# serenedb/serenedb

Measured on AMD Instinct MI355X. Metric: docs scored/sec BM25 top-1000 (+ rows/sec filter-agg), higher is better.
Workload: dtype f32; 1 GPU; bm25_top1000_4term_or_100M; execution=pipelined-batch, doc_count=100000000, k=1000, seed=43, postings_per_query=18005713, total_matches=17052989, parallelism=doc-range shards x1, RCCL allgather merge

## Files before the change

### serenedb_amd/csrc/hip/sdb_gpu.hip

```cpp

#include <hip/hip_runtime.h>

#include <algorithm>
#include <cfloat>
#include <cmath>
#include <cstdint>
#include <cstdlib>
#include <cstring>
#include <vector>
#include <chrono>
#include <cstdio>

#include "../../../include/sdb_gpu.h"
#include "sdb_internal.h"

#define SDB_TERM_SLOTS 64u
#ifndef SDB_WIN_DOCS
#define SDB_WIN_DOCS 24576u
#endif
#ifndef SDB_NTHREADS
#define SDB_NTHREADS 1024u
#endif
#define SDB_NWAVES (SDB_NTHREADS / 64u)
#define SDB_MAX_TERMS 32u
// ... 934 lines not shown
    }
    __syncthreads();
    SDB_T(4)
#endif
  }
  if (tid == 0 && wg_matches) atomicAdd(a.total_matches, wg_matches);
#ifdef SDB_TIMING
  if (tid == 0)
    for (int i = 0; i < 6; ++i)
      atomicAdd(&a.bucket_out[i], t_acc[i]);
#endif
}


struct SweepItem {
  uint32_t t;
  float num;
  const uint8_t* pl;
  SdbBlockDesc d;
};

template <uint32_t WD, uint32_t NTH, bool WIDE>
__launch_bounds__(NTH, NTH == 1024 ? 4 : 2) __global__
void topk_sweep_kernel(WindowArgs a, const TermDev* __restrict__ terms) {
  constexpr uint32_t NW = NTH / 64u;
  constexpr uint32_t NWORDS = WD / 64u;
  static_assert(WD - 1u < SDB_SLOT_ABSENT, "slot offsets are u16");
  extern __shared__ __attribute__((aligned(16))) char smem[];
  float* swin = (float*)smem;
  unsigned long long* mwin = (unsigned long long*)(swin + WD);
  uint32_t* scratch = (uint32_t*)(mwin + NWORDS);
  uint32_t* hist = scratch + NW * 384;
  uint32_t* shared_misc = hist + SDB_HIST_BINS;
  uint32_t* cursors = shared_misc + 2 + NW;
  float* wub = (float*)(cursors + SDB_MAX_TERMS);
  uint32_t* icnt = (uint32_t*)(wub + SDB_MAX_TERMS);
  uint32_t* iadv = icnt + SDB_MAX_TERMS;
  TermDev* tstage = (TermDev*)(iadv + SDB_MAX_TERMS);
  unsigned long long* lbuck =
    (unsigned long long*)(tstage + a.nterms);
  SdbBlockDesc* dcache =
    (SdbBlockDesc*)(lbuck + (a.fcol ? 2 * SDB_MAX_BUCKETS : 0u));
  const uint32_t stage_off =
    ((uint32_t)((char*)(dcache + a.nterms * a.dcache_n) - smem) + 15u) & ~15u;
  char* stage = smem + stage_off;
  const uint32_t C = a.round_items;

  const uint32_t tid = threadIdx.x;
  const int lane = tid & 63;
  const uint32_t wave = tid >> 6;
  for (uint32_t i = tid; i < a.nterms * (sizeof(TermDev) / 4); i += NTH)
    ((uint32_t*)tstage)[i] = ((const uint32_t*)terms)[i];
  const float inv_smax = (float)SDB_HIST_BINS / a.smax;
  uint32_t* gh = a.ghist + (blockIdx.x & 7u) * SDB_HIST_BINS;
  unsigned long long wg_matches = 0;
#ifdef SDB_TIMING
  unsigned long long t_acc[6] = {0, 0, 0, 0, 0, 0};
  long long t_mark = clock64();
#define SDB_TS(idx)                                        \
  if (tid == 0) {                                          \
    const long long now_ = clock64();                      \
    t_acc[idx] += (unsigned long long)(now_ - t_mark);     \
    t_mark = now_;                                         \
  }
#else
#define SDB_TS(idx)
#endif

  const uint32_t nwin = (a.doc_count + WD - 1) / WD;
  const uint32_t per = (nwin + gridDim.x - 1) / gridDim.x;
  const uint32_t w_lo = blockIdx.x * per;
  const uint32_t w_hi = min(nwin, w_lo + per);
  if (w_lo >= w_hi) return;

  __syncthreads();
  if (tid < a.nterms) {
    const TermDev te = tstage[tid];
    const uint32_t first_lo = 1u + w_lo * WD;
    cursors[tid] = (uint32_t)(
      lower_bound_last_doc(a.desc, te.desc_begin, te.desc_end, first_lo) -
      te.desc_begin);
  }
  __syncthreads();
  const float nc = tstage[0].nc, nl = tstage[0].nl;

  for (uint32_t w = w_lo; w < w_hi; ++w) {
    const uint32_t lo = 1u + w * WD;
    if (lo > a.doc_count) break;
    const uint32_t hi = min(lo + WD - 1u, a.doc_count);
    const uint32_t wlen = hi - lo + 1u;
    const bool derive = ((w & 3u) == 0) || (w < w_lo + 2);
    uint32_t my_excl_snap = 0;

    for (uint32_t t = wave; t < a.nterms; t += NW) {
      const TermDev te = tstage[t];
      uint64_t b = te.desc_begin + cursors[t] + (uint32_t)lane;
      uint32_t cnt = 0, adv = 0;
      for (;;) {
        uint32_t prev = 0xFFFFFFFFu, last = 0xFFFFFFFFu;
        if (b < te.desc_end) {
          prev = a.desc[b].prev_doc;
          last = a.desc[b].last_doc;
        }
        const uint32_t c = (uint32_t)__popcll(__ballot(prev < hi));
        adv += (uint32_t)__popcll(__ballot(last <= hi));
        cnt += c;
        if (c < 64u) break;
        b += 64u;
      }
      if (lane == 0) {
        icnt[t] = cnt;
        iadv[t] = adv;
      }
    }

    for (uint32_t i = tid; i < WD; i += NTH) swin[i] = 0.0f;
    for (uint32_t i = tid; i < NWORDS; i += NTH) mwin[i] = 0ull;
    if (derive)
      for (uint32_t i = tid; i < SDB_HIST_BINS; i += NTH) hist[i] = 0;
    if (a.fcol)
      for (uint32_t i = tid; i < 2 * a.nbuckets; i += NTH) lbuck[i] = 0;
    {
      const uint32_t words_per_term = a.dcache_n * 7u;
      for (uint32_t i = tid; i < a.nterms * words_per_term; i += NTH) {
        const uint32_t t = i / words_per_term;
        const uint32_t wrd = i % words_per_term;
        const TermDev te = tstage[t];
        const uint64_t b0 = te.desc_begin + cursors[t];
        const uint32_t avail =
          (uint32_t)(te.desc_end > b0 ? te.desc_end - b0 : 0);
        if (wrd < avail * 7u)
          ((uint32_t*)&dcache[t * a.dcache_n])[wrd] =
            ((const uint32_t*)&a.desc[b0])[wrd];
      }
    }
    if (tid == 0)
      shared_misc[0] = __hip_atomic_load(a.gthresh, __ATOMIC_RELAXED,
                                         __HIP_MEMORY_SCOPE_AGENT);
    if (a.wand) __syncthreads();
    if (a.wand) {
      for (uint32_t t = wave; t < a.nterms; t += NW) {
        const TermDev te = tstage[t];
        const uint32_t cur0w = cursors[t];
        float u = 0.0f;
        uint32_t beyond_f = 0;
        if ((uint32_t)lane < a.dcache_n &&
            te.desc_begin + cur0w + (uint32_t)lane < te.desc_end) {
          const SdbBlockDesc d = dcache[t * a.dcache_n + lane];
          if (d.prev_doc < hi)
            u = score_one(a.scorer, te.num, te.nc, te.nl, d.max_freq,
                          d.min_norm);
          else
            beyond_f = 1;
        }
#pragma unroll
        for (int o = 32; o; o >>= 1) u = fmaxf(u, __shfl_down(u, o, 64));
        const unsigned long long beyond = __ballot(beyond_f != 0);
        if (lane == 0) {
          float ub = u;
          if (!beyond) {
            for (uint64_t bb = te.desc_begin + cur0w + a.dcache_n;
                 bb < te.desc_end; ++bb) {
              const SdbBlockDesc d = a.desc[bb];
              if (d.prev_doc >= hi) break;
              const float uu = score_one(a.scorer, te.num, te.nc, te.nl,
                                         d.max_freq, d.min_norm);
              ub = uu > ub ? uu : ub;
            }
          }
          wub[t] = ub * a.fbmax * 1.0000019f;
        }
      }
    }
    __syncthreads();
    SDB_TS(0)
    float wand_total_ub = 0.0f;
    if (a.wand)
      for (uint32_t t = 0; t < a.nterms; ++t) wand_total_ub += wub[t];
    float gtw = 0.0f;
    if (a.wand && shared_misc[0]) {
      float t0 = (float)shared_misc[0] / inv_smax;
      uint32_t t0b;
      __builtin_memcpy(&t0b, &t0, 4);
      t0b = t0b > 2 ? t0b - 2 : 0;
      __builtin_memcpy(&gtw, &t0b, 4);
    }

    const uint32_t icnt_l = (uint32_t)lane < a.nterms ? icnt[lane] : 0u;
    const uint32_t ipre_incl = wave_incl_scan(icnt_l, lane);
    const uint32_t ipre_excl = ipre_incl - icnt_l;
    const uint32_t nitems =
      (uint32_t)__builtin_amdgcn_readlane((int)ipre_incl, 63);
    auto load_item = [&](uint32_t i, SweepItem& it) {
      const uint32_t t =
        (uint32_t)__builtin_ctzll(__ballot(ipre_incl > i));
      const uint32_t rel =
        i - (uint32_t)__builtin_amdgcn_readlane((int)ipre_excl, (int)t);
      const TermDev te = tstage[t];
      typedef __attribute__((address_space(3))) const uint32_t LdsWord;
      typedef __attribute__((address_space(1))) const uint32_t GlobalWord;
      uint32_t wv[10];
      if (rel < a.dcache_n) {
        LdsWord* p = (LdsWord*)&dcache[t * a.dcache_n + rel];
#pragma unroll
        for (int k = 0; k < 7; ++k) wv[k] = p[k];
      } else {
        GlobalWord* p =
          (GlobalWord*)&a.desc[te.desc_begin + cursors[t] + rel];
#pragma unroll
        for (int k = 0; k < 7; ++k) wv[k] = p[k];
      }
      __builtin_memcpy(wv + 7, &te.payload_begin, 8);
      __builtin_memcpy(wv + 9, &te.num, 4);
#pragma unroll
      for (int k = 0; k < 10; ++k)
        wv[k] = (uint32_t)__builtin_amdgcn_readfirstlane((int)wv[k]);
      uint64_t pbeg;
      __builtin_memcpy(&it.d, wv, 28);
      __builtin_memcpy(&pbeg, wv + 7, 8);
      __builtin_memcpy(&it.num, wv + 9, 4);
      it.t = t;
      it.pl = a.payload + pbeg;
// ... 90 lines not shown
        const uint32_t npair = (i1 - i0) * 64u;
        for (uint32_t p = tid; p < npair; p += NTH) {
          const char* sl = base + (p >> 6) * SDB_SLOT_BYTES;
          const uint32_t l = p & 63u;
          const float2 v = ((const float2*)sl)[l];
          const uint32_t o = ((const uint32_t*)(sl + 512))[l];
          const uint32_t o0 = o & 0xFFFFu, o1 = o >> 16;
          if (o0 != SDB_SLOT_ABSENT) swin_add(swin, o0, v.x);
          if (o1 != SDB_SLOT_ABSENT) swin_add(swin, o1, v.y);
        }
        __syncthreads();
      }
      SDB_TS(2)
    }
    if (tid < a.nterms) cursors[tid] += iadv[tid];

    uint32_t tbin_w = shared_misc[0];
    const uint32_t nw_act = (wlen + 63u) / 64u;
    uint32_t my_matches = 0;
    uint32_t my_cnt = 0;
    for (uint32_t i = tid; i < nw_act; i += NTH) {
      unsigned long long word = mwin[i];
      if (word && a.live) {
        const uint64_t d0 = (uint64_t)lo + 64u * i;
        const unsigned long long lw = (a.live[d0 >> 6] >> (d0 & 63u)) |
                                      (a.live[(d0 >> 6) + 1]
                                       << (64u - (d0 & 63u)));
        word &= lw;
        mwin[i] = word;
      }
      if (word && a.fcol) {
        unsigned long long w0 = word;
        while (w0) {
          const uint32_t bit = (uint32_t)__ffsll((long long)w0) - 1u;
          w0 &= w0 - 1;
          const uint32_t doc = lo + 64u * i + bit;
          const long long vv = a.fcol[doc];
          bool pass = vv >= a.flo && vv <= a.fhi;
          for (uint32_t x = 0; pass && x < a.nfx; ++x) {
            const long long xv = a.fxc[x][doc];
            if (a.fxop[x] == 1) pass = xv < a.fxlo[x];
            else if (a.fxop[x] == 2) pass = xv >= a.fxlo[x];
            else pass = (xv >= a.fxlo[x]) & (xv <= a.fxhi[x]);
          }
          if (!pass) {
            word &= ~(1ull << bit);
            continue;
          }
          const unsigned long long span_m1 =
            (unsigned long long)a.fhi - (unsigned long long)a.flo;
          const unsigned long long dv =
            (unsigned long long)vv - (unsigned long long)a.flo;
          const uint32_t bkt = WIDE
            ? sdb_bucket_wide(dv, a.nbuckets, span_m1)
            : sdb_bucket_narrow(dv, a.nbuckets, span_m1);
          atomicAdd(&lbuck[2 * bkt], 1ull);
          atomicAdd(&lbuck[2 * bkt + 1], (unsigned long long)vv);
        }
        mwin[i] = word;
      }
      if (!word) continue;
      my_matches += (uint32_t)__popcll(word);
      const uint32_t base = i * 64u;
      do {
        const uint32_t off = base + (uint32_t)__ffsll((long long)word) - 1u;
        word &= word - 1;
        const uint32_t sb = score_bin(swin[off], inv_smax);
        my_cnt += sb >= tbin_w ? 1u : 0u;
        if (derive) atomicAdd(&hist[sb], 1u);
      } while (word);
    }
    {
      const uint32_t incl0 = wave_incl_scan(my_cnt, lane);
      if (lane == 63) scratch[NTH + wave] = incl0;
      my_excl_snap = incl0 - my_cnt;
    }
    uint32_t wm = my_matches;
#pragma unroll
    for (int off = 32; off; off >>= 1) wm += __shfl_down(wm, off, 64);
    if (lane == 0) shared_misc[2 + wave] = wm;
    __syncthreads();
    SDB_TS(3)

    if (a.fcol)
      for (uint32_t i = tid; i < 2 * a.nbuckets; i += NTH)
        if (lbuck[i]) atomicAdd(&a.bucket_out[i], lbuck[i]);

    const uint32_t known_bin = __hip_atomic_load(
      a.gthresh, __ATOMIC_RELAXED, __HIP_MEMORY_SCOPE_AGENT);
    if (derive)
      for (uint32_t b = tid; b < SDB_HIST_BINS; b += NTH)
        if (b >= known_bin && hist[b]) atomicAdd(&gh[b], hist[b]);
    if (derive && wave == 0) {
      uint32_t part = 0;
      if (SDB_HIST_BINS - 1 - 4 * (uint32_t)lane + 3 >= known_bin) {
#pragma unroll
        for (int j = 0; j < 4; ++j) {
          const uint32_t b = SDB_HIST_BINS - 4 * lane - 4 + j;
#pragma unroll
          for (int sh = 0; sh < 8; ++sh)
            part += __hip_atomic_load(&a.ghist[sh * SDB_HIST_BINS + b],
                                      __ATOMIC_RELAXED,
                                      __HIP_MEMORY_SCOPE_AGENT);
        }
      }
      const uint32_t suff_incl = wave_incl_scan(part, lane);
      const uint32_t suff_prev = __shfl_up(suff_incl, 1, 64);
      const bool winner =
        suff_incl >= a.k && (lane == 0 || suff_prev < a.k);
      if (winner) {
        uint32_t cum = suff_incl - part;
        uint32_t binfloor = 0;
        for (int b = (int)(SDB_HIST_BINS - 1 - 4 * lane);; --b) {
          uint32_t add = 0;
#pragma unroll
          for (int sh = 0; sh < 8; ++sh)
            add += __hip_atomic_load(&a.ghist[sh * SDB_HIST_BINS + b],
                                     __ATOMIC_RELAXED,
                                     __HIP_MEMORY_SCOPE_AGENT);
          cum += add;
          if (cum >= a.k) {
            binfloor = (uint32_t)b;
            break;
          }
        }
        if (binfloor > known_bin) atomicMax(a.gthresh, binfloor);
      }
    }
    if (wave == 0 && lane == 0) {
      uint32_t total_m = 0;
      for (uint32_t v = 0; v < NW; ++v) total_m += shared_misc[2 + v];
      wg_matches += total_m;
    }
    SDB_TS(4)

    if (w == w_lo) {
      if (tid == 0)
        shared_misc[0] = __hip_atomic_load(a.gthresh, __ATOMIC_RELAXED,
                                           __HIP_MEMORY_SCOPE_AGENT);
      __syncthreads();
      tbin_w = shared_misc[0];
      uint32_t cnt2 = 0;
      for (uint32_t i = tid; i < nw_act; i += NTH) {
        unsigned long long word = mwin[i];
        if (!word) continue;
        const uint32_t base = i * 64u;
        do {
          const uint32_t off =
            base + (uint32_t)__ffsll((long long)word) - 1u;
          word &= word - 1;
          cnt2 += score_bin(swin[off], inv_smax) >= tbin_w ? 1u : 0u;
        } while (word);
      }
      const uint32_t incl2 = wave_incl_scan(cnt2, lane);
      if (lane == 63) scratch[NTH + wave] = incl2;
      my_excl_snap = incl2 - cnt2;
      __syncthreads();
    }

    uint32_t wave_base = 0;
    for (uint32_t v = 0; v < wave; ++v) wave_base += scratch[NTH + v];
    const uint32_t my_excl = wave_base + my_excl_snap;
    uint32_t block_total = 0;
    for (uint32_t v = 0; v < NW; ++v) block_total += scratch[NTH + v];
    if (tid == 0)
      shared_misc[1] =
        block_total ? atomicAdd(a.cand_count, block_total) : 0u;
    __syncthreads();
    const uint32_t cbase = shared_misc[1];
    if (cbase + block_total > a.cand_cap) {
      if (tid == 0) atomicExch(a.overflow, 1u);
      return;
    }
    uint32_t pos = cbase + my_excl;
    if (block_total)
      for (uint32_t i = tid; i < nw_act; i += NTH) {
        unsigned long long word = mwin[i];
        if (!word) continue;
        const uint32_t base = i * 64u;
        do {
          const uint32_t off =
            base + (uint32_t)__ffsll((long long)word) - 1u;
          word &= word - 1;
          const float s = swin[off];
          if (score_bin(s, inv_smax) >= tbin_w) {
            a.cands[pos].score = s;
            a.cands[pos].doc = lo + off;
            a.cands[pos].segment_idx = a.seg_idx;
            ++pos;
          }
        } while (word);
      }
    __syncthreads();
    SDB_TS(5)
  }
  if (tid == 0 && wg_matches) atomicAdd(a.total_matches, wg_matches);
#ifdef SDB_TIMING
  if (tid == 0)
    for (int i = 0; i < 6; ++i) atomicAdd(&a.bucket_out[i], t_acc[i]);
#endif
#undef SDB_TS
}



#ifndef SDB_PW_SUBW
#define SDB_PW_SUBW 1024u
#endif
#define SDB_PW_TERMS 4u
#define SDB_PW_NTH 256u

#ifndef SDB_PW_RING
#define SDB_PW_RING 256u
#endif
#ifndef SDB_PW_MINW
#define SDB_PW_MINW 2
#endif
#define SDB_PW_DSTAGE 8u
#define SDB_PW_WAVE_LDS_BYTES                                            \
  (SDB_PW_SUBW * 4  + (SDB_PW_SUBW / 64) * 8  +          \
   SDB_PW_TERMS * SDB_PW_RING * 8  + 384 * 4  +      \
   SDB_HIST_BINS * 4  +                                          \
   SDB_PW_TERMS * SDB_PW_DSTAGE * 28  + 32 )

struct PwState {
  uint64_t cur;
  uint64_t dend;
  uint64_t dsbase;
  uint64_t pbase;
  uint32_t ring_head;
  uint32_t ring_cnt;
  uint32_t cov;
  float num, nc, nl;
};

__device__ __forceinline__ uint32_t pw_fill_block(
  const WindowArgs& a, PwState& st, const SdbBlockDesc& d, int lane,
  uint32_t range_lo, uint32_t range_hi, unsigned long long* ring,
  uint32_t* scratch) {
  const uint8_t* pl = a.payload + st.pbase;
  uint32_t doc0 = 0, doc1 = 0;
  float s0 = 0.f, s1 = 0.f;
  bool have01 = false;
  if ((d.flags & 1u) && a.norm_stream) {
    const uint8_t* db = pl + d.doc_off;
    const uint8_t* fb = pl + d.freq_off;
    {
      const uint32_t dbits = (d.flags >> 1) & 31u;
      const uint32_t fbits = (d.flags >> 6) & 31u;
      const uint32_t nbits = (d.flags >> 11) & 31u;
      const uint8_t* nb = fb + 1 + 16u * fbits;
// ... 414 lines not shown
  const uint64_t b = b0 + blockIdx.x;
  if (blockIdx.x >= nblocks) return;
  const int lane = threadIdx.x & 63;
  const SdbBlockDesc d = desc[b];
  const uint8_t* pl = payload + payload_begin;
  decode_doc_block_wave(pl + d.doc_off, d.len, d.prev_doc, lane, dbuf);
  decode_freq_block_wave(pl + d.freq_off, d.len, lane, fbuf);
  __syncthreads();
  const uint64_t out0 = (uint64_t)blockIdx.x * 128u;
  for (uint32_t i = lane; i < d.len; i += 64) {
    docs[out0 + i] = dbuf[i];
    freqs[out0 + i] = fbuf[i];
  }
}

namespace {

struct SweepGeom {
  uint32_t wd, nth;
};

bool launch_sweep(const SweepGeom& g, bool wide, dim3 grid, size_t lds,
                  hipStream_t st, const WindowArgs& a,
                  const TermDev* terms) {
#define SDB_SWEEP_CASE(WDV, NTHV)                                          \
  if (g.wd == WDV && g.nth == NTHV) {                                      \
    if (wide)                                                              \
      hipLaunchKernelGGL((topk_sweep_kernel<WDV, NTHV, true>), grid,       \
                         dim3(NTHV), lds, st, a, terms);                   \
    else                                                                   \
      hipLaunchKernelGGL((topk_sweep_kernel<WDV, NTHV, false>), grid,      \
                         dim3(NTHV), lds, st, a, terms);                   \
    return true;                                                           \
  }
  SDB_SWEEP_CASE(24576, 1024)
  SDB_SWEEP_CASE(16384, 1024)
  SDB_SWEEP_CASE(12288, 512)
  SDB_SWEEP_CASE(8192, 512)
  SDB_SWEEP_CASE(8192, 256)
  SDB_SWEEP_CASE(4096, 256)
  SDB_SWEEP_CASE(24576, 512)
  SDB_SWEEP_CASE(32768, 512)
#undef SDB_SWEEP_CASE
  return false;
}

size_t sweep_lds_fixed(const SweepGeom& g, uint32_t nterms, bool hybrid) {
  return (size_t)g.wd * 4 + g.wd / 8 + (g.nth / 64) * 1536 +
         SDB_HIST_BINS * 4 + (2 + g.nth / 64) * 4 + 4 * SDB_MAX_TERMS * 4 +
         sizeof(TermDev) * nterms + (hybrid ? 16 * SDB_MAX_BUCKETS : 0);
}

struct SweepLds {
  bool ok;
  uint32_t dcache_n, round_items, wgs_per_cu;
  size_t bytes;
};
SweepLds plan_sweep_lds(const SweepGeom& g, uint32_t nterms, bool hybrid) {
  constexpr size_t kLds = 163840;
  const uint32_t nw = g.nth / 64u;
  const size_t fixed = sweep_lds_fixed(g, nterms, hybrid);
  auto total = [&](uint32_t dn, uint32_t c) {
    return fixed + sizeof(SdbBlockDesc) * dn * nterms + 16  +
           (size_t)c * SDB_SLOT_BYTES;
  };
  SweepLds p{false, SDB_DESC_CACHE, nw, 1, 0};
  while (p.dcache_n > 1 && total(p.dcache_n, nw) > kLds) --p.dcache_n;
  if (total(p.dcache_n, nw) > kLds) return p;
  const uint32_t wgs = std::min<uint32_t>(
    (uint32_t)(kLds / total(p.dcache_n, nw)), 32u / nw);
  const uint32_t want = g.wd / 512u + nterms;
  const uint32_t fit =
    (uint32_t)((kLds / wgs - total(p.dcache_n, 0)) / SDB_SLOT_BYTES);
  p.round_items = std::max(nw, std::min(want, fit));
  if (const char* e = getenv("SDB_SWEEP_ROUND_ITEMS")) {
    const unsigned long v = strtoul(e, nullptr, 10);
    if (v >= 1 && v < p.round_items)
      p.round_items = std::max<uint32_t>(nw, (uint32_t)v);
  }
  p.bytes = total(p.dcache_n, p.round_items);
  p.wgs_per_cu = wgs;
  p.ok = true;
  return p;
}

int check_gpu() {
  int n = 0;
  hipError_t e = hipGetDeviceCount(&n);
  if (e != hipSuccess || n == 0) return SDB_ERR_NO_GPU;
  return SDB_OK;
}

int parse_blob(const void* blob, size_t size, SdbSegHeader* hdr_out) {
  if (!blob || size < sizeof(SdbSegHeader)) return -51;
  SdbSegHeader hdr;
  std::memcpy(&hdr, blob, sizeof(hdr));
  if (hdr.magic != SDB_SEG_MAGIC) return -52;
  if (hdr.version < 1 || hdr.version > 3 || hdr.version == 2)
    return -53;
  if (hdr.blob_size > size) return -54;
  const uint64_t bs = hdr.blob_size;
  if (hdr.off_terms > bs ||
      (uint64_t)hdr.nterms * sizeof(SdbTermEntry) > bs - hdr.off_terms)
    return SDB_ERR_BAD_SEGMENT;
  if (hdr.off_desc > bs ||
      hdr.total_blocks > (bs - hdr.off_desc) / sizeof(SdbBlockDesc))
    return SDB_ERR_BAD_SEGMENT;
  if (hdr.off_norms > bs ||
      ((uint64_t)hdr.doc_count + 1) * 4 > bs - hdr.off_norms)
    return SDB_ERR_BAD_SEGMENT;
  if (hdr.off_payload > bs || hdr.payload_size > bs - hdr.off_payload)
    return SDB_ERR_BAD_SEGMENT;
  *hdr_out = hdr;
  return SDB_OK;
}

}

extern "C" {

const char* sdb_gpu_version(void) { return "sdb_gpu 0.1 gfx950"; }

static void ctx_free_partial(SdbGpuCtx* ctx) {
  if (ctx->d_scan_out) (void)hipFree(ctx->d_scan_out);
  if (ctx->d_scan_passed) (void)hipFree(ctx->d_scan_passed);
  if (ctx->d_cands) (void)hipFree(ctx->d_cands);
  if (ctx->d_cands2) (void)hipFree(ctx->d_cands2);
  if (ctx->d_ghist2) (void)hipFree(ctx->d_ghist2);
  if (ctx->d_qmisc) (void)hipFree(ctx->d_qmisc);
  if (ctx->h_qmisc) (void)hipHostFree(ctx->h_qmisc);
  if (ctx->h_terms_pin) (void)hipHostFree(ctx->h_terms_pin);
  if (ctx->h_cands_pin) (void)hipHostFree(ctx->h_cands_pin);
  if (ctx->copy_stream) (void)hipStreamDestroy(ctx->copy_stream);
  if (ctx->d_cand_count) (void)hipFree(ctx->d_cand_count);
  if (ctx->d_total_matches) (void)hipFree(ctx->d_total_matches);
  if (ctx->d_gthresh) (void)hipFree(ctx->d_gthresh);
  if (ctx->d_ghist) (void)hipFree(ctx->d_ghist);
  if (ctx->d_buckets) (void)hipFree(ctx->d_buckets);
  if (ctx->d_terms) (void)hipFree(ctx->d_terms);
  if (ctx->d_overflow) (void)hipFree(ctx->d_overflow);
  if (ctx->h_counts) (void)hipHostFree(ctx->h_counts);
  if (ctx->h_matches) (void)hipHostFree(ctx->h_matches);
  if (ctx->stream) (void)hipStreamDestroy(ctx->stream);
  delete ctx;
}

#define CTX_CHECK(x)                                   \
  do {                                                 \
    hipError_t _e = (x);                               \
    if (_e != hipSuccess) {                            \
      ctx_free_partial(ctx);                           \
      return _e == hipErrorNoDevice ? SDB_ERR_NO_GPU   \
             : _e == hipErrorOutOfMemory ? SDB_ERR_OOM \
                                         : SDB_ERR_HIP; \
    }                                                  \
  } while (0)

int sdb_gpu_ctx_create(int device, SdbGpuCtx** out) {
  if (!out) return SDB_ERR_INVALID;
  int rc = check_gpu();
  if (rc) return rc;
  HIP_CHECK(hipSetDevice(device));
  auto* ctx = new SdbGpuCtx{};
  ctx->device = device;
  CTX_CHECK(hipStreamCreate(&ctx->stream));
  CTX_CHECK(hipStreamCreate(&ctx->copy_stream));
// ... 360 lines not shown
    const uint32_t slot = s % SDB_TERM_SLOTS;
    if (s && slot == 0) HIP_CHECK(hipStreamSynchronize(ctx->stream));
    TermDev* d_tslot = ctx->d_terms + (size_t)slot * SDB_MAX_TERMS;
    TermDev* tdev = ctx->h_terms_pin + (size_t)slot * SDB_MAX_TERMS;
    for (uint32_t t = 0; t < plan->nterms; ++t) {
      const SdbTermEntry& te = seg->terms_host[plan->terms[t].term_idx];
      tdev[t].desc_begin = te.desc_begin;
      tdev[t].desc_end = te.desc_end;
      tdev[t].payload_begin = te.payload_begin;
      tdev[t].num = num[t];
      tdev[t].nc = nc;
      tdev[t].nl = nl;
    }
    HIP_CHECK(hipMemcpyAsync(d_tslot, tdev, sizeof(TermDev) * plan->nterms,
                             hipMemcpyHostToDevice, ctx->stream));
    WindowArgs a{};
    a.fcol = hybrid ? seg->fcols[hpreds[0].slot] : nullptr;
    a.flo = hybrid ? hpreds[0].lo : 0;
    a.fhi = hybrid ? hpreds[0].hi : 0;
    a.nfx = hybrid ? nhp - 1 : 0;
    for (uint32_t x = 0; hybrid && x + 1 < nhp; ++x) {
      a.fxc[x] = seg->fcols[hpreds[x + 1].slot];
      a.fxop[x] = (int)hpreds[x + 1].op;
      a.fxlo[x] = hpreds[x + 1].lo;
      a.fxhi[x] = hpreds[x + 1].hi;
    }
    a.nbuckets = h_nbuckets;
    a.bucket_out = ctx->d_buckets;
    a.desc = seg->desc;
    a.payload = seg->payload;
    a.norms = seg->norms;
    a.doc_count = seg->hdr.doc_count;
    a.scorer = scorer;
    a.wand = (plan->wand && (plan->min_match <= 1) && !hybrid) ? 1u : 0u;
    a.count_only = count_only;
    a.norm_stream = seg->hdr.version >= 3 ? 1u : 0u;
    a.nterms = plan->nterms;
    a.min_match = plan->min_match ? plan->min_match : 1;
    a.k = k;
    a.smax = smax;
    a.seg_idx = s;
    a.dcache_n = dcache_n;
    a.fb = plan->filter_boost ? seg->fboost : nullptr;
    a.fbmax = plan->filter_boost ? fbmax : 1.0f;
    a.live = seg->live;
    a.gthresh = ctx->d_gthresh;
    a.ghist = ctx->d_ghist;
    a.cands = ctx->d_cands;
    a.cand_count = ctx->d_cand_count;
    a.cand_cap = SDB_CAND_CAP;
    a.total_matches = ctx->d_total_matches;
    a.overflow = ctx->d_overflow;
    if (use_wave) {
      const uint32_t nwaves = (uint32_t)std::min<uint64_t>(
        4096, ((uint64_t)seg->hdr.doc_count + SDB_PW_SUBW - 1) /
                SDB_PW_SUBW);
      const uint32_t rdocs =
        (uint32_t)(((uint64_t)seg->hdr.doc_count + nwaves - 1) / nwaves);
      const size_t pw_lds = (size_t)(SDB_PW_NTH / 64) *
                            SDB_PW_WAVE_LDS_BYTES;
      if (s == 0 && k != 0xFFFFFFFFu && nwaves > 64) {
        WindowArgs sa = a;
        sa.ghist = ctx->d_ghist + 8 * SDB_HIST_BINS;
        const uint32_t seed_waves = 256;
        const uint32_t seed_docs = 4096;
        const uint32_t seed_stride = (uint32_t)std::max<uint64_t>(
          seed_docs, seg->hdr.doc_count / seed_waves);
        hipLaunchKernelGGL(topk_wave_kernel,
                           dim3((seed_waves + 3) / 4), dim3(SDB_PW_NTH),
                           pw_lds, ctx->stream, sa, d_tslot, seed_waves,
                           seed_docs, seed_stride, 1);
        HIP_CHECK(hipGetLastError());
      }
      hipLaunchKernelGGL(topk_wave_kernel, dim3((nwaves + 3) / 4),
                         dim3(SDB_PW_NTH), pw_lds, ctx->stream, a,
                         d_tslot, nwaves, rdocs, rdocs, 0);
      HIP_CHECK(hipGetLastError());
      continue;
    }
    if (use_sweep) {
      a.dcache_n = slds.dcache_n;
      a.round_items = slds.round_items;
      const uint32_t nwin = (seg->hdr.doc_count + sgeom.wd - 1) / sgeom.wd;
      uint32_t ngrid = 256u * slds.wgs_per_cu;
      if (ngrid > nwin) ngrid = nwin;
      if (!launch_sweep(sgeom, wide_span, dim3(ngrid), slds.bytes,
                        ctx->stream, a, d_tslot))
        return SDB_ERR_INVALID;
      HIP_CHECK(hipGetLastError());
      continue;
    }
    const uint32_t nwin =
      (seg->hdr.doc_count + SDB_WIN_DOCS - 1) / SDB_WIN_DOCS;
    uint32_t wgs_per_cu = (uint32_t)(163840 / lds_bytes);
    if (wgs_per_cu < 1) wgs_per_cu = 1;
    if (wgs_per_cu > 4) wgs_per_cu = 4;
    uint32_t ngrid = 256u * wgs_per_cu;
    if (ngrid > nwin) ngrid = nwin;
    if (wide_span)
      hipLaunchKernelGGL(topk_window_kernel<true>, dim3(ngrid),
                         dim3(SDB_NTHREADS), lds_bytes, ctx->stream, a,
                         d_tslot);
    else
      hipLaunchKernelGGL(topk_window_kernel<false>, dim3(ngrid),
                         dim3(SDB_NTHREADS), lds_bytes, ctx->stream, a,
                         d_tslot);
    HIP_CHECK(hipGetLastError());
  }

  HIP_CHECK(hipEventRecord(ctx->ev_b, ctx->stream));

  HIP_CHECK(hipMemcpyAsync(ctx->h_counts, ctx->d_cand_count, 4,
                           hipMemcpyDeviceToHost, ctx->stream));
  HIP_CHECK(hipMemcpyAsync(ctx->h_counts + 1, ctx->d_overflow, 4,
                           hipMemcpyDeviceToHost, ctx->stream));
  HIP_CHECK(hipMemcpyAsync(ctx->h_counts + 2, ctx->d_gthresh, 4,
                           hipMemcpyDeviceToHost, ctx->stream));
  HIP_CHECK(hipMemcpyAsync(ctx->h_matches, ctx->d_total_matches, 8,
                           hipMemcpyDeviceToHost, ctx->stream));
  HIP_CHECK(hipStreamSynchronize(ctx->stream));
  {
    float ms = 0.0f;
    HIP_CHECK(hipEventElapsedTime(&ms, ctx->ev_a, ctx->ev_b));
    ctx->last_kernel_ms = (double)ms;
  }
  if (ctx->h_counts[1]) return SDB_ERR_OOM;
  const uint32_t ncand = ctx->h_counts[0];
  ctx->last_ncand = ncand;
  if (!hits) {
    *out_count = 0;
    *total_matches = *ctx->h_matches;
    ctx->last_gtau = 0.0f;
    return SDB_OK;
  }
  const auto t_rb0 = std::chrono::steady_clock::now();
  std::vector<SdbScoreDoc> cands_heap;
  SdbScoreDoc* cands = ctx->h_cands_pin;
  if (ncand && ncand <= SDB_PIN_CANDS) {
    HIP_CHECK(hipMemcpyAsync(ctx->h_cands_pin, ctx->d_cands,
                             sizeof(SdbScoreDoc) * ncand,
                             hipMemcpyDeviceToHost, ctx->stream));
    HIP_CHECK(hipStreamSynchronize(ctx->stream));
  } else if (ncand) {
    cands_heap.resize(ncand);
    HIP_CHECK(hipMemcpy(cands_heap.data(), ctx->d_cands,
                        sizeof(SdbScoreDoc) * ncand, hipMemcpyDeviceToHost));
    cands = cands_heap.data();
  }
  ctx->last_readback_ms =
    std::chrono::duration<double, std::milli>(
      std::chrono::steady_clock::now() - t_rb0)
      .count();
  const auto t_sel0 = std::chrono::steady_clock::now();
  const uint32_t final_bin = ctx->h_counts[2];
  const float inv_smax = (float)SDB_HIST_BINS / smax;
  size_t n = 0;
  for (size_t i = 0; i < ncand; ++i) {
    const float s = cands[i].score;
    if (sdb_host_score_bin(s, inv_smax) >= final_bin && s > FLT_MIN)
      cands[n++] = cands[i];
  }
  const float gtau_final =
    final_bin ? (float)final_bin / inv_smax : 0.0f;
  auto cmp = [](const SdbScoreDoc& x, const SdbScoreDoc& y) {
    if (x.score != y.score) return x.score > y.score;
    if (x.segment_idx != y.segment_idx) return x.segment_idx < y.segment_idx;
    return x.doc < y.doc;
  };
  const size_t kk = std::min<size_t>(k, n);
  if (kk < n) std::nth_element(cands, cands + kk, cands + n, cmp);
  std::sort(cands, cands + kk, cmp);
  std::copy(cands, cands + kk, hits);
  *out_count = (uint32_t)kk;
  *total_matches = *ctx->h_matches;
#ifdef SDB_TIMING
  {
    unsigned long long tdbg[6];
    hipMemcpy(tdbg, ctx->d_buckets, 48, hipMemcpyDeviceToHost);
    fprintf(stderr,
            use_sweep
              ? "[timing cyc/WG avg] zero+stage=%llu stage1=%llu stage2=%llu "
                "sweep=%llu tau=%llu append=%llu\n"
              : "[timing cyc/WG avg] zero+stage=%llu phases=%llu hist=%llu "
                "tau=%llu append=%llu term0=%llu\n",
            tdbg[0] / 256, tdbg[1] / 256, tdbg[2] / 256, tdbg[3] / 256,
            tdbg[4] / 256, tdbg[5] / 256);
  }
#endif
  if (hybrid && bucket_count && bucket_sum) {
    std::vector<unsigned long long> hb(2 * h_nbuckets);
    HIP_CHECK(hipMemcpy(hb.data(), ctx->d_buckets, 8ull * 2 * h_nbuckets,
                        hipMemcpyDeviceToHost));
    for (uint32_t i = 0; i < h_nbuckets; ++i) {
      bucket_count[i] = (int64_t)hb[2 * i];
      bucket_sum[i] = (int64_t)hb[2 * i + 1];
    }
  }
  ctx->last_gtau = gtau_final;
  ctx->last_select_ms =
    std::chrono::duration<double, std::milli>(
      std::chrono::steady_clock::now() - t_sel0)
      .count();
  return SDB_OK;
}

int sdb_gpu_execute_topk(SdbGpuCtx* ctx, SdbGpuSegment* const* segs,
                         uint32_t nsegs, const SdbQueryPlan* plan, uint32_t k,
                         SdbScoreDoc* hits, uint32_t* out_count,
                         uint64_t* total_matches) {
  return exec_topk_impl(ctx, segs, nsegs, plan, k, 0, nullptr, 0, 0,
                        nullptr,
                        nullptr, hits, out_count, total_matches);
}

static int exec_topk_batch_impl(
  SdbGpuCtx* ctx, SdbGpuSegment* const* segs, uint32_t nsegs,
  const SdbQueryPlan* plan, uint32_t k, uint32_t nq,
  const SdbHybridPred* hpreds, uint32_t nhp, uint32_t h_nbuckets,
  int64_t* bucket_counts, int64_t* bucket_sums, SdbScoreDoc* hits,
  uint32_t* out_counts, uint64_t* totals) {
  if (!ctx || !segs || !plan || !plan->terms || !hits || !out_counts ||
      !totals || nq == 0 || plan->nterms == 0 ||
      plan->nterms > SDB_MAX_TERMS || k == 0 || k == 0xFFFFFFFFu)
    return SDB_ERR_INVALID;
  const bool hybrid = nhp > 0;
  if (hybrid) {
    if (!hpreds || nhp > SDB_MAX_FILTER_COLS ||
        hpreds[0].op != SDB_PRED_BETWEEN || h_nbuckets == 0 ||
        h_nbuckets > SDB_MAX_BUCKETS || !bucket_counts || !bucket_sums)
      return SDB_ERR_INVALID;
    for (uint32_t x = 0; x < nhp; ++x) {
      if (hpreds[x].slot >= 4 ||
          (hpreds[x].op != SDB_PRED_LT && hpreds[x].op != SDB_PRED_GE &&
           hpreds[x].op != SDB_PRED_BETWEEN))
        return SDB_ERR_INVALID;
      for (uint32_t sx = 0; sx < nsegs; ++sx)
        if (!segs[sx]->fcols[hpreds[x].slot]) return SDB_ERR_INVALID;
    }
  }
  for (uint32_t i = 0; i < plan->nterms; ++i) {
    for (uint32_t j = i + 1; j < plan->nterms; ++j)
      if (plan->terms[i].term_idx == plan->terms[j].term_idx)
        return SDB_ERR_INVALID;
    if (!(plan->terms[i].boost >= 0.0f)) return SDB_ERR_INVALID;
  }
  PlanStats ps;
  {
    const int prc = prep_plan_stats(segs, nsegs, plan, 0, &ps);
    if (prc) return prc;
  }
  const float smax = ps.smax;
  const float inv_smax = (float)SDB_HIST_BINS / smax;

  const bool wide_span =
    hybrid && sdb_bucket_span_wide((unsigned long long)hpreds[0].hi -
                                     (unsigned long long)hpreds[0].lo,
                                   h_nbuckets);

  SweepGeom sgeom{24576, 1024};
  bool use_sweep = plan->min_match <= 1;
  bool use_wave = false;
  if (const char* e = getenv("SDB_TOPK_PATH")) {
    if (!strcmp(e, "wave"))
      use_wave = use_sweep && plan->nterms <= SDB_PW_TERMS &&
                 !plan->wand && !hybrid;
// ... 47 lines not shown
                             4 * SDB_HIST_BINS * 16, ctx->stream));
    if (hybrid)
      HIP_CHECK(hipMemsetAsync(
        ctx->d_buckets + (size_t)qs * 2 * SDB_MAX_BUCKETS, 0,
        8 * 2 * SDB_MAX_BUCKETS, ctx->stream));
    for (uint32_t sg = 0; sg < nsegs; ++sg) {
      SdbGpuSegment* seg = segs[sg];
      const uint32_t slot = (q * nsegs + sg) % SDB_TERM_SLOTS;
      if ((q * nsegs + sg) >= SDB_TERM_SLOTS && slot == 0)
        HIP_CHECK(hipStreamSynchronize(ctx->stream));
      TermDev* d_tslot = ctx->d_terms + (size_t)slot * SDB_MAX_TERMS;
      TermDev* tdev = ctx->h_terms_pin + (size_t)slot * SDB_MAX_TERMS;
      for (uint32_t t = 0; t < plan->nterms; ++t) {
        const SdbTermEntry& te = seg->terms_host[plan->terms[t].term_idx];
        tdev[t].desc_begin = te.desc_begin;
        tdev[t].desc_end = te.desc_end;
        tdev[t].payload_begin = te.payload_begin;
        tdev[t].num = ps.num[t];
        tdev[t].nc = ps.nc;
        tdev[t].nl = ps.nl;
      }
      HIP_CHECK(hipMemcpyAsync(d_tslot, tdev,
                               sizeof(TermDev) * plan->nterms,
                               hipMemcpyHostToDevice, ctx->stream));
      WindowArgs a{};
      a.desc = seg->desc;
      a.payload = seg->payload;
      a.norms = seg->norms;
      a.doc_count = seg->hdr.doc_count;
      a.scorer = plan->scorer;
      a.wand = (plan->wand && plan->min_match <= 1 && !hybrid) ? 1u : 0u;
      a.norm_stream = seg->hdr.version >= 3 ? 1u : 0u;
      a.nterms = plan->nterms;
      a.min_match = plan->min_match ? plan->min_match : 1;
      a.k = k;
      a.smax = smax;
      a.seg_idx = sg;
      a.cand_cap = SDB_CAND_CAP;
      a.fcol = hybrid ? seg->fcols[hpreds[0].slot] : nullptr;
      a.flo = hybrid ? hpreds[0].lo : 0;
      a.fhi = hybrid ? hpreds[0].hi : 0;
      a.nfx = hybrid ? nhp - 1 : 0;
      for (uint32_t x = 0; hybrid && x + 1 < nhp; ++x) {
        a.fxc[x] = seg->fcols[hpreds[x + 1].slot];
        a.fxop[x] = (int)hpreds[x + 1].op;
        a.fxlo[x] = hpreds[x + 1].lo;
        a.fxhi[x] = hpreds[x + 1].hi;
      }
      a.nbuckets = hybrid ? h_nbuckets : 0;
      a.bucket_out = ctx->d_buckets + (size_t)qs * 2 * SDB_MAX_BUCKETS;
      a.fb = plan->filter_boost ? seg->fboost : nullptr;
      a.fbmax = ps.fbmax;
      a.live = seg->live;
      set_ptrs(qs, a);
      if (use_wave) {
        const uint32_t nwaves = (uint32_t)std::min<uint64_t>(
          4096, ((uint64_t)seg->hdr.doc_count + SDB_PW_SUBW - 1) /
                  SDB_PW_SUBW);
        const uint32_t rdocs =
          (uint32_t)(((uint64_t)seg->hdr.doc_count + nwaves - 1) / nwaves);
        const size_t pw_lds =
          (size_t)(SDB_PW_NTH / 64) * SDB_PW_WAVE_LDS_BYTES;
        if (sg == 0 && nwaves > 64) {
          WindowArgs sa = a;
          sa.ghist = a.ghist + 8 * SDB_HIST_BINS;
          hipLaunchKernelGGL(topk_wave_kernel, dim3(64), dim3(SDB_PW_NTH),
                             pw_lds, ctx->stream, sa, d_tslot, 256, 4096,
                             (uint32_t)std::max<uint64_t>(
                               4096, seg->hdr.doc_count / 256),
                             1);
          HIP_CHECK(hipGetLastError());
        }
        hipLaunchKernelGGL(topk_wave_kernel, dim3((nwaves + 3) / 4),
                           dim3(SDB_PW_NTH), pw_lds, ctx->stream, a,
                           d_tslot, nwaves, rdocs, rdocs, 0);
        HIP_CHECK(hipGetLastError());
        continue;
      }
      if (use_sweep) {
        a.dcache_n = slds.dcache_n;
        a.round_items = slds.round_items;
        const uint32_t nwin =
          (seg->hdr.doc_count + sgeom.wd - 1) / sgeom.wd;
        uint32_t ngrid = 256u * slds.wgs_per_cu;
        if (ngrid > nwin) ngrid = nwin;
        if (!launch_sweep(sgeom, wide_span, dim3(ngrid), slds.bytes,
                          ctx->stream, a, d_tslot))
          return SDB_ERR_INVALID;
        HIP_CHECK(hipGetLastError());
        continue;
      }
      a.dcache_n = gen_dcache_n;
      const uint32_t nwin =
        (seg->hdr.doc_count + SDB_WIN_DOCS - 1) / SDB_WIN_DOCS;
      uint32_t wgs_per_cu =
        (uint32_t)(163840 /
                   (lds_fixed_gen +
                    sizeof(SdbBlockDesc) * gen_dcache_n * plan->nterms));
      if (wgs_per_cu < 1) wgs_per_cu = 1;
      if (wgs_per_cu > 4) wgs_per_cu = 4;
      uint32_t ngrid = 256u * wgs_per_cu;
      if (ngrid > nwin) ngrid = nwin;
      const size_t gen_lds =
        lds_fixed_gen + sizeof(SdbBlockDesc) * gen_dcache_n * plan->nterms;
      if (wide_span)
        hipLaunchKernelGGL(topk_window_kernel<true>, dim3(ngrid),
                           dim3(SDB_NTHREADS), gen_lds, ctx->stream, a,
                           d_tslot);
      else
        hipLaunchKernelGGL(topk_window_kernel<false>, dim3(ngrid),
                           dim3(SDB_NTHREADS), gen_lds, ctx->stream, a,
                           d_tslot);
      HIP_CHECK(hipGetLastError());
    }
    HIP_CHECK(hipMemcpyAsync(ctx->h_qmisc + 512 * qs,
                             ctx->d_qmisc + 512 * qs, 512,
                             hipMemcpyDeviceToHost, ctx->stream));
    HIP_CHECK(hipEventRecord(ctx->ev_q[qs], ctx->stream));
    return SDB_OK;
  };

  auto harvest = [&](uint32_t q) -> int {
    const int qs = (int)(q & 1u);
    HIP_CHECK(hipEventSynchronize(ctx->ev_q[qs]));
    const unsigned char* m = ctx->h_qmisc + 512 * qs;
    uint32_t final_bin, ncand, ovf;
    uint64_t total;
    std::memcpy(&final_bin, m + 0, 4);
    std::memcpy(&ncand, m + 128, 4);
    std::memcpy(&ovf, m + 256, 4);
    std::memcpy(&total, m + 384, 8);
    if (ovf) return SDB_ERR_OOM;
    SdbScoreDoc* csrc = qs ? ctx->d_cands2 : ctx->d_cands;
    std::vector<SdbScoreDoc> heap_c;
    SdbScoreDoc* cands;
    if (ncand <= SDB_PIN_CANDS) {
      HIP_CHECK(hipMemcpyAsync(ctx->h_cands_pin, csrc,
                               sizeof(SdbScoreDoc) * ncand,
                               hipMemcpyDeviceToHost, ctx->copy_stream));
      HIP_CHECK(hipStreamSynchronize(ctx->copy_stream));
      cands = ctx->h_cands_pin;
    } else {
      heap_c.resize(ncand);
      HIP_CHECK(hipMemcpyAsync(heap_c.data(), csrc,
                               sizeof(SdbScoreDoc) * ncand,
                               hipMemcpyDeviceToHost, ctx->copy_stream));
      HIP_CHECK(hipStreamSynchronize(ctx->copy_stream));
      cands = heap_c.data();
    }
    size_t n = 0;
    for (size_t i = 0; i < ncand; ++i) {
      const float sc = cands[i].score;
      if (sdb_host_score_bin(sc, inv_smax) >= final_bin && sc > FLT_MIN)
        cands[n++] = cands[i];
    }
    auto cmp = [](const SdbScoreDoc& x, const SdbScoreDoc& y) {
      if (x.score != y.score) return x.score > y.score;
      if (x.segment_idx != y.segment_idx)
        return x.segment_idx < y.segment_idx;
      return x.doc < y.doc;
    };
    const size_t kk = std::min<size_t>(k, n);
    if (kk < n) std::nth_element(cands, cands + kk, cands + n, cmp);
    std::sort(cands, cands + kk, cmp);
    std::copy(cands, cands + kk, hits + (size_t)q * k);
    out_counts[q] = (uint32_t)kk;
    totals[q] = total;
    if (hybrid) {
// ... 134 lines not shown
                          0, nullptr, nullptr, nullptr, &dummy_n,
                          total_matches);
  if (rc) return rc;
  const uint32_t ncand = ctx->last_ncand;
  std::vector<SdbScoreDoc> cands(ncand);
  if (ncand)
    HIP_CHECK(hipMemcpy(cands.data(), ctx->d_cands,
                        sizeof(SdbScoreDoc) * ncand, hipMemcpyDeviceToHost));
  std::sort(cands.begin(), cands.end(),
            [](const SdbScoreDoc& x, const SdbScoreDoc& y) {
              return x.doc < y.doc;
            });
  const uint64_t n = std::min<uint64_t>(cap, cands.size());
  for (uint64_t i = 0; i < n; ++i) docs_out[i] = cands[i].doc;
  if (col_out && seg->fcols[0] && n) {
    uint32_t* d_docs;
    long long* d_vals;
    HIP_CHECK(hipMalloc(&d_docs, 4 * n));
    HIP_CHECK(hipMalloc(&d_vals, 8 * n));
    HIP_CHECK(hipMemcpy(d_docs, docs_out, 4 * n, hipMemcpyHostToDevice));
    const uint32_t nb = (uint32_t)((n + 255) / 256);
    hipLaunchKernelGGL(gather_col_kernel, dim3(nb), dim3(256), 0,
                       ctx->stream, d_docs, seg->fcols[0], d_vals, n);
    HIP_CHECK(hipGetLastError());
    HIP_CHECK(hipMemcpyAsync(col_out, d_vals, 8 * n, hipMemcpyDeviceToHost,
                             ctx->stream));
    HIP_CHECK(hipStreamSynchronize(ctx->stream));
    (void)hipFree(d_docs);
    (void)hipFree(d_vals);
  }
  *out_count = n;
  return SDB_OK;
}

int sdb_gpu_decode_term(SdbGpuCtx* ctx, SdbGpuSegment* seg, uint32_t term_idx,
                        uint32_t* docs, uint32_t* freqs) {
  if (!ctx || !seg || !docs || !freqs || term_idx >= seg->hdr.nterms)
    return SDB_ERR_INVALID;
  const SdbTermEntry& te = seg->terms_host[term_idx];
  const uint64_t nblocks = te.desc_end - te.desc_begin;
  if (!nblocks) return SDB_OK;
  uint32_t *d_docs, *d_freqs;
  const uint64_t cap = nblocks * 128;
  HIP_CHECK(hipMalloc(&d_docs, cap * 4));
  HIP_CHECK(hipMalloc(&d_freqs, cap * 4));
  hipLaunchKernelGGL(decode_term_kernel, dim3((uint32_t)nblocks), dim3(64), 0,
                     ctx->stream, seg->desc, te.desc_begin, nblocks,
                     seg->payload, te.payload_begin, d_docs, d_freqs);
  HIP_CHECK(hipGetLastError());
  HIP_CHECK(hipStreamSynchronize(ctx->stream));
  std::vector<uint32_t> tmp_d(cap), tmp_f(cap);
  HIP_CHECK(hipMemcpy(tmp_d.data(), d_docs, cap * 4, hipMemcpyDeviceToHost));
  HIP_CHECK(hipMemcpy(tmp_f.data(), d_freqs, cap * 4, hipMemcpyDeviceToHost));
  (void)hipFree(d_docs);
  (void)hipFree(d_freqs);
  uint32_t n = 0;
  for (uint64_t b = 0; b < nblocks; ++b) {
    const uint32_t len =
      (b + 1 == nblocks) ? (te.df - (uint32_t)(nblocks - 1) * 128u) : 128u;
    std::memcpy(docs + n, tmp_d.data() + b * 128, len * 4);
    std::memcpy(freqs + n, tmp_f.data() + b * 128, len * 4);
    n += len;
  }
  return SDB_OK;
}

int sdb_gpu_last_kernel_ms(SdbGpuCtx* ctx, double* ms) {
  if (!ctx || !ms) return SDB_ERR_INVALID;
  *ms = ctx->last_kernel_ms;
  return SDB_OK;
}

int sdb_gpu_last_stats(SdbGpuCtx* ctx, double* kernel_ms, unsigned* ncand,
                       float* gtau, double* readback_ms, double* select_ms) {
  if (!ctx) return SDB_ERR_INVALID;
  if (kernel_ms) *kernel_ms = ctx->last_kernel_ms;
  if (ncand) *ncand = ctx->last_ncand;
  if (gtau) *gtau = ctx->last_gtau;
  if (readback_ms) *readback_ms = ctx->last_readback_ms;
  if (select_ms) *select_ms = ctx->last_select_ms;
  return SDB_OK;
}

}
```

### serenedb_amd/csrc/hip/sdb_internal.h

```cpp
#pragma once
#include <hip/hip_runtime.h>
#include "../../../include/sdb_gpu.h"

struct TermDev {
  uint64_t desc_begin;
  uint64_t desc_end;
  uint64_t payload_begin;
  float num;
  float nc;
  float nl;
};

__host__ __device__ inline bool sdb_bucket_span_wide(
  unsigned long long span_m1, uint32_t nb) {
  return nb != 0 && (span_m1 == ~0ull || span_m1 > ~0ull / nb);
}

__host__ __device__ inline uint32_t sdb_bucket_narrow(
  unsigned long long d, uint32_t nb, unsigned long long span_m1) {
  uint32_t bkt = (uint32_t)((d * nb) / (span_m1 + 1ull));
  if (bkt >= nb) bkt = nb - 1;
  return bkt;
}

__host__ __device__ inline unsigned long long sdb_mul64hi(
  unsigned long long x, unsigned long long y) {
#if defined(__HIP_DEVICE_COMPILE__)
  return __umul64hi(x, y);
#else
  return (unsigned long long)(((unsigned __int128)x * y) >> 64);
#endif
}

__host__ __device__ inline uint32_t sdb_bucket_wide(
  unsigned long long d, uint32_t nb, unsigned long long span_m1) {
  const unsigned long long nhi = sdb_mul64hi(d, nb), nlo = d * nb;
  if (span_m1 == ~0ull) return (uint32_t)nhi;
  const unsigned long long span = span_m1 + 1ull;
  uint32_t q = 0;
  for (uint32_t step = 64; step; step >>= 1) {
    const uint32_t c = q + step;
    if (c >= nb) continue;
    const unsigned long long chi = sdb_mul64hi(c, span), clo = c * span;
    if (chi < nhi || (chi == nhi && clo <= nlo)) q = c;
  }
  return q;
}

struct SdbGpuCtx {
  int device;
  hipStream_t stream;
  unsigned long long* d_scan_out;
  uint64_t scan_out_cap;
  unsigned long long* d_scan_passed;
  SdbScoreDoc* d_cands;
  uint32_t* d_cand_count;
  unsigned long long* d_total_matches;
  uint32_t* d_gthresh;
  uint32_t* d_ghist;
  unsigned long long* d_buckets;
  TermDev* d_terms;
  uint32_t* d_overflow;
  uint32_t* h_counts;
  unsigned long long* h_matches;
  hipEvent_t ev_a, ev_b;
  hipStream_t copy_stream;
  SdbScoreDoc* d_cands2;
  uint32_t* d_ghist2;
  unsigned char* d_qmisc;
  unsigned char* h_qmisc;
  TermDev* h_terms_pin;
  SdbScoreDoc* h_cands_pin;
  hipEvent_t ev_q[2];
  double last_kernel_ms;
  unsigned last_ncand;
  float last_gtau;
  double last_readback_ms;
  double last_select_ms;
  unsigned long long* d_topn_hist;
  void* d_topn_cand;
  uint64_t topn_cand_cap;
  uint32_t* d_topn_rg;
  uint64_t topn_rg_cap;
};
```

Before: 56.36 billion docs/s.

## Prefetch next window's block descriptors during tail phase and dedicate threshold wave

Hoists the per-term block-descriptor counting and dcache staging out of the window loop top into a lambda. It runs once before the loop and then, for the next window, on waves other than the threshold wave while the current window's tail work proceeds. Wave 1 alone does the global histogram read and threshold update, and the candidate reservation atomic is moved earlier. The winning-bin search now uses the per-lane bin sums instead of re-reading global histograms. This removes a barrier and overlaps global descriptor loads with histogram and threshold work, at the cost of more control complexity and a threshold snapshot that is one step staler. An env override for sweep grid size is also added.

```diff
diff --git a/serenedb_amd/csrc/hip/sdb_gpu.hip b/serenedb_amd/csrc/hip/sdb_gpu.hip
--- a/serenedb_amd/csrc/hip/sdb_gpu.hip
+++ b/serenedb_amd/csrc/hip/sdb_gpu.hip
@@ -1040,17 +1040,11 @@
       te.desc_begin);
   }
   __syncthreads();
-  const float nc = tstage[0].nc, nl = tstage[0].nl;
-
-  for (uint32_t w = w_lo; w < w_hi; ++w) {
-    const uint32_t lo = 1u + w * WD;
-    if (lo > a.doc_count) break;
-    const uint32_t hi = min(lo + WD - 1u, a.doc_count);
-    const uint32_t wlen = hi - lo + 1u;
-    const bool derive = ((w & 3u) == 0) || (w < w_lo + 2);
-    uint32_t my_excl_snap = 0;
-
-    for (uint32_t t = wave; t < a.nterms; t += NW) {
+
+  auto fetch_window = [&](uint32_t hi_n, uint32_t w0) {
+    if (wave < w0) return;
+    const uint32_t nwv = NW - w0;
+    for (uint32_t t = wave - w0; t < a.nterms; t += nwv) {
       const TermDev te = tstage[t];
       uint64_t b = te.desc_begin + cursors[t] + (uint32_t)lane;
       uint32_t cnt = 0, adv = 0;
@@ -1060,8 +1054,8 @@
           prev = a.desc[b].prev_doc;
           last = a.desc[b].last_doc;
         }
-        const uint32_t c = (uint32_t)__popcll(__ballot(prev < hi));
-        adv += (uint32_t)__popcll(__ballot(last <= hi));
+        const uint32_t c = (uint32_t)__popcll(__ballot(prev < hi_n));
+        adv += (uint32_t)__popcll(__ballot(last <= hi_n));
         cnt += c;
         if (c < 64u) break;
         b += 64u;
@@ -1071,6 +1065,35 @@
         iadv[t] = adv;
       }
     }
+    const uint32_t words_per_term = a.dcache_n * 7u;
+    for (uint32_t i = tid - w0 * 64u; i < a.nterms * words_per_term;
+         i += nwv * 64u) {
+      const uint32_t t = i / words_per_term;
+      const uint32_t wrd = i % words_per_term;
+      const TermDev te = tstage[t];
+      const uint64_t b0 = te.desc_begin + cursors[t];
+      const uint32_t avail =
+        (uint32_t)(te.desc_end > b0 ? te.desc_end - b0 : 0);
+      if (wrd < avail * 7u)
+        ((uint32_t*)&dcache[t * a.dcache_n])[wrd] =
+          ((const uint32_t*)&a.desc[b0])[wrd];
+    }
+  };
+  fetch_window((uint32_t)min((uint64_t)(w_lo + 1u) * WD,
+                             (uint64_t)a.doc_count), 0);
+  if (tid == 0)
+    shared_misc[0] = __hip_atomic_load(a.gthresh, __ATOMIC_RELAXED,
+                                       __HIP_MEMORY_SCOPE_AGENT);
+  __syncthreads();
+  const float nc = tstage[0].nc, nl = tstage[0].nl;
+
+  for (uint32_t w = w_lo; w < w_hi; ++w) {
+    const uint32_t lo = 1u + w * WD;
+    if (lo > a.doc_count) break;
+    const uint32_t hi = min(lo + WD - 1u, a.doc_count);
+    const uint32_t wlen = hi - lo + 1u;
+    const bool derive = ((w & 3u) == 0) || (w < w_lo + 2);
+    uint32_t my_excl_snap = 0;
 
     for (uint32_t i = tid; i < WD; i += NTH) swin[i] = 0.0f;
     for (uint32_t i = tid; i < NWORDS; i += NTH) mwin[i] = 0ull;
@@ -1078,24 +1101,6 @@
       for (uint32_t i = tid; i < SDB_HIST_BINS; i += NTH) hist[i] = 0;
     if (a.fcol)
       for (uint32_t i = tid; i < 2 * a.nbuckets; i += NTH) lbuck[i] = 0;
-    {
-      const uint32_t words_per_term = a.dcache_n * 7u;
-      for (uint32_t i = tid; i < a.nterms * words_per_term; i += NTH) {
-        const uint32_t t = i / words_per_term;
-        const uint32_t wrd = i % words_per_term;
-        const TermDev te = tstage[t];
-        const uint64_t b0 = te.desc_begin + cursors[t];
-        const uint32_t avail =
-          (uint32_t)(te.desc_end > b0 ? te.desc_end - b0 : 0);
-        if (wrd < avail * 7u)
-          ((uint32_t*)&dcache[t * a.dcache_n])[wrd] =
-            ((const uint32_t*)&a.desc[b0])[wrd];
-      }
-    }
-    if (tid == 0)
-      shared_misc[0] = __hip_atomic_load(a.gthresh, __ATOMIC_RELAXED,
-                                         __HIP_MEMORY_SCOPE_AGENT);
-    if (a.wand) __syncthreads();
     if (a.wand) {
       for (uint32_t t = wave; t < a.nterms; t += NW) {
         const TermDev te = tstage[t];
@@ -1352,49 +1357,75 @@
     __syncthreads();
     SDB_TS(3)
 
+    constexpr uint32_t DRV = 1;
+    const bool first = w == w_lo;
+    uint32_t block_total = 0, wave_base = 0, resv = 0;
+    auto count_and_reserve = [&]() {
+      for (uint32_t v = 0; v < NW; ++v) {
+        const uint32_t c = scratch[NTH + v];
+        block_total += c;
+        wave_base += v < wave ? c : 0u;
+      }
+      if (tid == 0 && block_total)
+        resv = atomicAdd(a.cand_count, block_total);
+    };
+    if (!first) count_and_reserve();
+    if (w + 1 < w_hi) fetch_window(hi + min(WD, a.doc_count - hi), DRV + 1);
+
     if (a.fcol)
       for (uint32_t i = tid; i < 2 * a.nbuckets; i += NTH)
         if (lbuck[i]) atomicAdd(&a.bucket_out[i], lbuck[i]);
 
-    const uint32_t known_bin = __hip_atomic_load(
-      a.gthresh, __ATOMIC_RELAXED, __HIP_MEMORY_SCOPE_AGENT);
     if (derive)
       for (uint32_t b = tid; b < SDB_HIST_BINS; b += NTH)
-        if (b >= known_bin && hist[b]) atomicAdd(&gh[b], hist[b]);
-    if (derive && wave == 0) {
-      uint32_t part = 0;
-      if (SDB_HIST_BINS - 1 - 4 * (uint32_t)lane + 3 >= known_bin) {
+        if (b >= tbin_w && hist[b]) atomicAdd(&gh[b], hist[b]);
+
+    uint32_t snap_next = tbin_w;
+    if (wave == DRV) {
+      uint32_t gth = tbin_w;
+      if (!first)
+        gth = __hip_atomic_load(a.gthresh, __ATOMIC_RELAXED,
+                                __HIP_MEMORY_SCOPE_AGENT);
+      uint32_t binfloor = 0;
+      bool winner = false;
+      if (derive) {
+        uint32_t bsum[4] = {0, 0, 0, 0};
+        if (SDB_HIST_BINS - 1 - 4 * (uint32_t)lane + 3 >= tbin_w) {
 #pragma unroll
-        for (int j = 0; j < 4; ++j) {
-          const uint32_t b = SDB_HIST_BINS - 4 * lane - 4 + j;
+          for (int j = 0; j < 4; ++j) {
+            const uint32_t b = SDB_HIST_BINS - 4 * lane - 4 + j;
 #pragma unroll
-          for (int sh = 0; sh < 8; ++sh)
-            part += __hip_atomic_load(&a.ghist[sh * SDB_HIST_BINS + b],
-                                      __ATOMIC_RELAXED,
-                                      __HIP_MEMORY_SCOPE_AGENT);
-        }
-      }
-      const uint32_t suff_incl = wave_incl_scan(part, lane);
-      const uint32_t suff_prev = __shfl_up(suff_incl, 1, 64);
-      const bool winner =
-        suff_incl >= a.k && (lane == 0 || suff_prev < a.k);
-      if (winner) {
-        uint32_t cum = suff_incl - part;
-        uint32_t binfloor = 0;
-        for (int b = (int)(SDB_HIST_BINS - 1 - 4 * lane);; --b) {
-          uint32_t add = 0;
+            for (int sh = 0; sh < 8; ++sh)
+              bsum[j] += __hip_atomic_load(&a.ghist[sh * SDB_HIST_BINS + b],
+                                           __ATOMIC_RELAXED,
+                                           __HIP_MEMORY_SCOPE_AGENT);
+          }
+        }
+        const uint32_t part = bsum[0] + bsum[1] + bsum[2] + bsum[3];
+        const uint32_t suff_incl = wave_incl_scan(part, lane);
+        const uint32_t suff_prev = __shfl_up(suff_incl, 1, 64);
+        winner = suff_incl >= a.k && (lane == 0 || suff_prev < a.k);
+        if (winner) {
+          uint32_t cum = suff_incl - part;
 #pragma unroll
-          for (int sh = 0; sh < 8; ++sh)
-            add += __hip_atomic_load(&a.ghist[sh * SDB_HIST_BINS + b],
-                                     __ATOMIC_RELAXED,
-                                     __HIP_MEMORY_SCOPE_AGENT);
-          cum += add;
-          if (cum >= a.k) {
-            binfloor = (uint32_t)b;
-            break;
+          for (int j = 3; j >= 0; --j) {
+            const bool below = cum < a.k;
+            cum += bsum[j];
+            if (below && cum >= a.k)
+              binfloor = SDB_HIST_BINS - 4 * (uint32_t)lane - 4 + (uint32_t)j;
           }
-        }
-        if (binfloor > known_bin) atomicMax(a.gthresh, binfloor);
+          if (binfloor > gth) atomicMax(a.gthresh, binfloor);
+        }
+      }
+      if (first) {
+        if (lane == 0)
+          shared_misc[0] = __hip_atomic_load(a.gthresh, __ATOMIC_RELAXED,
+                                             __HIP_MEMORY_SCOPE_AGENT);
+      } else {
+        uint32_t nb = winner && binfloor > gth ? binfloor : gth;
+        const unsigned long long wmask = __ballot(winner);
+        if (wmask) nb = __shfl(nb, (int)__builtin_ctzll(wmask), 64);
+        snap_next = nb;
       }
     }
     if (wave == 0 && lane == 0) {
@@ -1402,12 +1433,8 @@
       for (uint32_t v = 0; v < NW; ++v) total_m += shared_misc[2 + v];
       wg_matches += total_m;
     }
-    SDB_TS(4)
-
-    if (w == w_lo) {
-      if (tid == 0)
-        shared_misc[0] = __hip_atomic_load(a.gthresh, __ATOMIC_RELAXED,
-                                           __HIP_MEMORY_SCOPE_AGENT);
+
+    if (first) {
       __syncthreads();
       tbin_w = shared_misc[0];
       uint32_t cnt2 = 0;
@@ -1426,17 +1453,15 @@
       if (lane == 63) scratch[NTH + wave] = incl2;
       my_excl_snap = incl2 - cnt2;
       __syncthreads();
-    }
-
-    uint32_t wave_base = 0;
-    for (uint32_t v = 0; v < wave; ++v) wave_base += scratch[NTH + v];
+      count_and_reserve();
+    }
+    if (tid == 0) shared_misc[1] = resv;
+    __syncthreads();
+    SDB_TS(4)
+
+    if (!first && tid == DRV * 64u) shared_misc[0] = snap_next;
+
     const uint32_t my_excl = wave_base + my_excl_snap;
-    uint32_t block_total = 0;
-    for (uint32_t v = 0; v < NW; ++v) block_total += scratch[NTH + v];
-    if (tid == 0)
-      shared_misc[1] =
-        block_total ? atomicAdd(a.cand_count, block_total) : 0u;
-    __syncthreads();
     const uint32_t cbase = shared_misc[1];
     if (cbase + block_total > a.cand_cap) {
       if (tid == 0) atomicExch(a.overflow, 1u);
@@ -2017,6 +2042,16 @@
   p.wgs_per_cu = wgs;
   p.ok = true;
   return p;
+}
+
+uint32_t sweep_grid(const SweepLds& p, uint32_t nwin) {
+  uint32_t ngrid = 256u * p.wgs_per_cu;
+  if (const char* e = getenv("SDB_SWEEP_GRID")) {
+    char* end = nullptr;
+    const unsigned long v = strtoul(e, &end, 10);
+    if (end != e && *end == '\0' && v >= 1 && v < ngrid) ngrid = (uint32_t)v;
+  }
+  return std::min(ngrid, nwin);
 }
 
 int check_gpu() {
@@ -2543,8 +2578,8 @@
       a.dcache_n = slds.dcache_n;
       a.round_items = slds.round_items;
       const uint32_t nwin = (seg->hdr.doc_count + sgeom.wd - 1) / sgeom.wd;
-      uint32_t ngrid = 256u * slds.wgs_per_cu;
-      if (ngrid > nwin) ngrid = nwin;
+      const uint32_t ngrid = sweep_grid(slds, nwin);
+      ctx->last_sweep_grid = ngrid;
       if (!launch_sweep(sgeom, wide_span, dim3(ngrid), slds.bytes,
                         ctx->stream, a, d_tslot))
         return SDB_ERR_INVALID;
@@ -2640,8 +2675,8 @@
     hipMemcpy(tdbg, ctx->d_buckets, 48, hipMemcpyDeviceToHost);
     fprintf(stderr,
             use_sweep
-              ? "[timing cyc/WG avg] zero+stage=%llu stage1=%llu stage2=%llu "
-                "sweep=%llu tau=%llu append=%llu\n"
+              ? "[timing cyc/WG avg] zero=%llu stage1=%llu stage2=%llu "
+                "sweep=%llu tail=%llu append=%llu\n"
               : "[timing cyc/WG avg] zero+stage=%llu phases=%llu hist=%llu "
                 "tau=%llu append=%llu term0=%llu\n",
             tdbg[0] / 256, tdbg[1] / 256, tdbg[2] / 256, tdbg[3] / 256,
@@ -2855,8 +2890,8 @@
         a.round_items = slds.round_items;
         const uint32_t nwin =
           (seg->hdr.doc_count + sgeom.wd - 1) / sgeom.wd;
-        uint32_t ngrid = 256u * slds.wgs_per_cu;
-        if (ngrid > nwin) ngrid = nwin;
+        const uint32_t ngrid = sweep_grid(slds, nwin);
+        ctx->last_sweep_grid = ngrid;
         if (!launch_sweep(sgeom, wide_span, dim3(ngrid), slds.bytes,
                           ctx->stream, a, d_tslot))
           return SDB_ERR_INVALID;
@@ -3157,4 +3192,10 @@
   return SDB_OK;
 }
 
-}
+int sdb_gpu_last_sweep_grid(SdbGpuCtx* ctx, unsigned* grid) {
+  if (!ctx || !grid) return SDB_ERR_INVALID;
+  *grid = ctx->last_sweep_grid;
+  return SDB_OK;
+}
+
+}
diff --git a/serenedb_amd/csrc/hip/sdb_internal.h b/serenedb_amd/csrc/hip/sdb_internal.h
--- a/serenedb_amd/csrc/hip/sdb_internal.h
+++ b/serenedb_amd/csrc/hip/sdb_internal.h
@@ -74,6 +74,7 @@
   hipEvent_t ev_q[2];
   double last_kernel_ms;
   unsigned last_ncand;
+  unsigned last_sweep_grid;
   float last_gtau;
   double last_readback_ms;
   double last_select_ms;
```

Measured after the change: 61.10 billion docs/s, median of 6. 1.08x the previous value.
